# caki35/UNet-Torch

Measured on AMD Instinct MI355X. Metric: images/sec training step, 4-level U-Net 1ch→2cls 512×512, at 1/2/4/8 MI355X, higher is better.
Workload: dtype f16

## Files before the change

include/unetmi.h:

```cpp
#ifndef UNETMI_H
#define UNETMI_H
#include <stddef.h>
#include <stdint.h>

#ifdef __cplusplus
extern "C" {
#endif

typedef void* umi_stream_t;

enum { UMI_F32 = 0, UMI_F16 = 1 };
enum { UMI_OK = 0, UMI_ERR_BADARG = -1, UMI_ERR_UNSUPPORTED = -2, UMI_ERR_WORKSPACE = -3 };
enum { UMI_CONV_UPSAMPLE2 = 1,
       UMI_CONV_FORCE_GENERIC = 2,
       UMI_CONV_DGRAD_STRIDED = 4,
       UMI_CONV_ACCUMULATE = 8,
       UMI_CONV_F32_MFMA = 16,
       UMI_CONV_F32_MFMA_1X1 = 32,
       UMI_CONV_F32_MFMA_2X2 = 64   };

int umi_version(void);
const char* umi_arch(void);

int umi_tune_conv3x3_impl(int impl);

int umi_pack_kn(const float* src, void* dst, int T, int K, int N, long st, long sk, long sn,
                int flip_t, int Kpad, int Npad, int dtype, umi_stream_t stream);

int umi_pack_kn8(const float* src, void* dst, int T, int K, int N, long st, long sk, long sn,
                 int flip_t, int Kpad, int Npad, int dtype, umi_stream_t stream);

int umi_conv_fwd(const void* x, int ldx, const void* tx, const void* wp, const float* bias,
                 void* y, int ldy, float* stat_part,
                 int N, int H, int W, int Ci, int Co, int R, int S, int stride, int pad,
                 int Ho, int Wo, int off_h, int off_w, int out_H, int out_W,
                 int in_dtype, int out_dtype, int flags, umi_stream_t stream);
int umi_linear_fused(const void* x, int ldx, const void* wp8, const float* bias, void* y, int ldy, long M, int Ci, int Co,
                     int epi, float p, unsigned seed, const unsigned* seed_dev, void* mask, const void* aux, int ldaux,
                     void* y2, int ldy2, int dtype, umi_stream_t stream);

int umi_conv_fwd_plan(int N, int H, int W, int Ci, int Co, int R, int S, int stride, int pad,
                      int ldx, int ldy, int in_dtype, int out_dtype, int flags, int has_bias,
                      int* layout, int* stat_rows);

int umi_bn_finalize(const float* stat_part, int rows, int C, double count,
                    const float* gamma, const float* beta, float eps, float momentum,
                    float* running_mean, float* running_var,
                    void* tx_out, float* rstd_out, umi_stream_t stream);
int umi_bn_stat_sums(const float* stat_part, int rows, int C, double* sums, umi_stream_t stream);
int umi_bn_finalize_sums(const double* sums, int C, double count,
                         const float* gamma, const float* beta, float eps, float momentum,
                         float* running_mean, float* running_var,
                         void* tx_out, float* rstd_out, umi_stream_t stream);

int umi_pool2_fwd(const void* x, int ldx, const void* tx, void* y, int ldy,
                  int N, int H, int W, int C, int dtype, umi_stream_t stream);
int umi_pool2_bwd(const void* dpool, int lddp, const void* x, int ldx, const void* tx,
                  void* da, int ldda, int accumulate,
                  int N, int H, int W, int C, int dtype, umi_stream_t stream);

size_t umi_bn_bwd_ws_bytes(long M, int C);
int umi_bn_bwd_reduce(const void* da, int ldda, const void* y, int ldy, const void* tx,
                      const float* rstd, float* sum_dz, float* sum_dzx,
                      long M, int C, int dtype, void* ws, size_t ws_bytes, umi_stream_t stream);
int umi_bn_bwd_apply(void* da, int ldda, const void* y, int ldy, const void* tx,
                     const float* rstd, const float* sum_dz, const float* sum_dzx,
                     long M, int C, int dtype, umi_stream_t stream);
int umi_bn_bwd_apply_count(void* da, int ldda, const void* y, int ldy, const void* tx,
                           const float* rstd, const float* sum_dz, const float* sum_dzx,
                           long M, long count, int C, int dtype, umi_stream_t stream);

int umi_conv_dgrad_bnred(const void* dy, int lddy, const void* wp8, void* da, int ldda, const void* ybn, int ldybn,
                         const void* txbn, const float* rstd, float* part, int N, int H, int W, int Ci, int Co,
                         int dtype, umi_stream_t stream);

int umi_conv_gather_bnred_rows(int N, int H, int W, int Ci, int Co, int R, int S, int stride, int pad, int Ho, int Wo,
                               int ldx, int ldy, int dtype, int flags);
int umi_conv_gather_bnred(const void* x, int ldx, const void* wp8, void* y, int ldy, const void* ybn, int ldybn,
                          const void* txbn, const float* rstd, float* part, int N, int H, int W, int Ci, int Co, int R, int S,
                          int stride, int pad, int Ho, int Wo, int dtype, int flags, umi_stream_t stream);

int umi_head_dgrad_bnred_rows(long P, int Ci, int Co, int ldda, int dtype);
int umi_head_dgrad_bnred(const void* dl, int lddl, const void* wp, void* da, int ldda, const void* ybn, int ldybn,
                         const void* txbn, const float* rstd, float* part, long P, int Ci, int Co, int dtype,
                         umi_stream_t stream);
size_t umi_head_bwd_fused_ws_bytes(long P, int Ci, int Co);
int umi_head_bwd_fused(const void* dl, int lddl, const void* wp, void* da, int ldda, const void* ybn, int ldybn,
                       const void* txbn, const float* rstd, float* part, float* dW, long s_co, long s_ci, float out_scale,
                       void* ws, size_t ws_bytes, long P, int Ci, int Co, int dtype, umi_stream_t stream);

int umi_conv3x3_fwd_act(const void* x, int ldx, const void* tx, const void* wp8, const void* out_tx, void* y, int ldy,
                        int N, int H, int W, int Ci, int Co, int dtype, umi_stream_t stream);
int umi_bn_stats_rows(long M, int C);
int umi_bn_stats(const void* x, int ldx, float* part, long M, int C, int dtype, umi_stream_t stream);
int umi_pool2_bwd_bnred_stat_rows(int N, int H, int W, int C);
int umi_pool2_bwd_bnred(const void* dpool, int lddp, const void* x, int ldx, const void* tx, const float* rstd, void* da,
                        int ldda, int accumulate, float* part, int N, int H, int W, int C, int dtype, umi_stream_t stream);
int umi_bn_bwd_from_partials(const float* part, int rows, int C, float* sum_dz, float* sum_dzx, umi_stream_t stream);

size_t umi_conv_wgrad_ws_bytes(int N, int Ho, int Wo, int Ci, int Co, int R, int S, int dtype, int flags);
int umi_conv_wgrad(const void* x, int ldx, const void* txa, const void* dy, int lddy, const void* txb,
                   float* dW, long s_co, long s_ci, long s_t, float out_scale,
                   int N, int H, int W, int Ci, int Co, int R, int S, int stride, int pad,
                   int Ho, int Wo, int dtype, int flags, void* ws, size_t ws_bytes, umi_stream_t stream);
typedef struct umi_wgrad_pending {
    const float* part;
    float* dW;
    long s_co, s_ci, s_t;
    float scale;
    int splits, RS, Ci, Co;
} umi_wgrad_pending;
int umi_conv_wgrad_deferred(const void* x, int ldx, const void* txa, const void* dy, int lddy, const void* txb,
                            float* dW, long s_co, long s_ci, long s_t, float out_scale, int N, int H, int W, int Ci, int Co,
                            int R, int S, int stride, int pad, int Ho, int Wo, int dtype, int flags, void* ws, size_t ws_bytes,
                            umi_wgrad_pending* out, umi_stream_t stream);
int umi_wgrad_reduce_group(int n, const void* items , umi_stream_t stream);
int umi_conv_wgrad_bias(const void* x, int ldx, const void* dy, int lddy, const void* txb, float* dW, long s_co, long s_ci,
                        long s_t, float* dbias, float out_scale, int N, int H, int W, int Ci, int Co, int Ho, int Wo, int dtype,
                        int flags, void* ws, size_t ws_bytes, umi_wgrad_pending* out, umi_stream_t stream);
int umi_conv_wgrad_group(int n, const void* const* x, int ldx, const void* const* dy, int lddy, float* const* dW, long s_co,
                         long s_ci, float out_scale, long M, int Ci, int Co, int dtype, umi_stream_t stream);
int umi_conv_wgrad_bnapply(const void* x, int ldx, const void* txa, const void* da, int ldda, const void* y, int ldy,
                           const void* tx_bn, const float* rstd, const float* sum_dz, const float* sum_dzx, void* dz,
                           int lddz, float* dW, long s_co, long s_ci, long s_t, float out_scale, int N, int H, int W,
                           int Ci, int Co, int R, int S, int stride, int pad, int dtype, int flags, void* ws,
                           size_t ws_bytes, umi_stream_t stream);
int umi_conv_wgrad_bnapply_count(const void* x, int ldx, const void* txa, const void* da, int ldda, const void* y, int ldy,
                                 const void* tx_bn, const float* rstd, const float* sum_dz, const float* sum_dzx, void* dz,
                                 int lddz, float* dW, long s_co, long s_ci, long s_t, float out_scale, int N, int H, int W,
                                 int Ci, int Co, int R, int S, int stride, int pad, int dtype, int flags, long count, void* ws,
                                 size_t ws_bytes, umi_stream_t stream);

size_t umi_colsum_ws_bytes(long M, int C);
int umi_colsum(const void* x, int ldx, float* out, float out_scale, long M, int C, int dtype,
               void* ws, size_t ws_bytes, umi_stream_t stream);
int umi_colsum_group(int n, const void* const* xs, int ldx, float* const* outs, float out_scale, long M, int C, int dtype,
                     void* ws, size_t ws_bytes, umi_stream_t stream);

int umi_materialize_nchw(const void* x, int ldx, const void* tx, float* y_nchw,
                         int N, int H, int W, int C, int dtype, umi_stream_t stream);


int umi_wstd_fwd(const float* w, float* wstd, float* rstd, int Co, int K, float eps, umi_stream_t stream);
int umi_wstd_bwd(const float* wstd, const float* rstd, const float* g, float* dw, int Co, int K, umi_stream_t stream);
typedef struct umi_wstd_desc {
    const float* w;
    float* ws;
    float* rstd;
    long off;
    int Co, K;
    float eps;
    int blk0;
    float* dw;
} umi_wstd_desc;
int umi_wstd_fwd_multi(const void* descs, int n_desc, int total_rows, umi_stream_t stream);
int umi_wstd_bwd_multi(const void* descs, int n_desc, int total_rows, const float* g_base, float* dw_base, umi_stream_t stream);

size_t umi_gn_fwd_ws_bytes(int N, long HW, int C);
int umi_gn_fwd(const void* x, int ldx, const float* gamma, const float* beta, const void* res, int ldr, void* y, int ldy,
               float* mean, float* rstd, int relu, int N, long HW, int C, int G, float eps, int dtype,
               void* ws, size_t ws_bytes, umi_stream_t stream);
size_t umi_gn_bwd_ws_bytes(int N, long HW, int C, int G);
int umi_gn_bwd(const void* dy, int lddy, const void* y, int ldy, const void* x, int ldx, const float* mean,
               const float* rstd, const float* gamma, int relu, void* dx, int lddx, void* dres, int lddr,
               float* dgamma, float* dbeta, float out_scale, int N, long HW, int C, int G, int dtype,
               void* ws, size_t ws_bytes, float* part_out, umi_stream_t stream);
int umi_gn_param_grads_group(int n, const float* const* parts, const int* Cs, int N, float* const* dgammas,
                             float* const* dbetas, float out_scale, umi_stream_t stream);

int umi_pool3s2_fwd(const void* x, int ldx, void* y, int ldy, void* idx, int N, int H, int W, int C, int dtype,
                    umi_stream_t stream);
int umi_pool3s2_bwd(const void* dy, int lddy, const void* x, int ldx, const void* idx, void* dx, int lddx, int N, int H, int W,
                    int C, int dtype, umi_stream_t stream);

int umi_ln_fwd(const void* x, int ldx, const float* gamma, const float* beta, void* y, int ldy, float* mean, float* rstd,
               long M, int C, float eps, int dtype, umi_stream_t stream);
size_t umi_ln_bwd_ws_bytes(long M, int C);
int umi_ln_bwd(const void* dy, int lddy, const void* x, int ldx, const float* gamma, const float* mean,
               const float* rstd, void* dx, int lddx, float* dgamma, float* dbeta, float out_scale, long M, int C,
               int dtype, void* ws, size_t ws_bytes, int* rows_out, umi_stream_t stream);

int umi_elementwise(int mode, const void* x, int ldx, const void* g, int ldg, void* y, int ldy, long M, int C,
                    long bcast_rows, int dtype, umi_stream_t stream);

int umi_dropout(const void* x, int ldx, void* y, int ldy, void* mask, int backward, float p, unsigned seed, long M, int C,
                int dtype, const void* tx, const unsigned* seed_dev, umi_stream_t stream);
int umi_dropout_fused(const void* x, int ldx, void* y, int ldy, void* mask, int backward, float p, unsigned seed, long M, int C,
                      int dtype, const unsigned* seed_dev, const void* aux, int ldaux, int gelu, umi_stream_t stream);

int umi_attn_fwd(const void* q, const void* k, const void* v, int ld, void* o, int ldo, float* lse, int B, int N, int heads,
                 int D, int dtype, umi_stream_t stream);
int umi_attn_bwd(const void* q, const void* k, const void* v, int ld, const void* o, const void* dO, int ldo,
                 const float* lse, void* dq, void* dk, void* dv, int ldd, float* delta, int B, int N, int heads, int D,
                 int dtype, umi_stream_t stream);
enum { UMI_ATTN_F32_MFMA = 1  };
int umi_attn_fwd_flags(const void* q, const void* k, const void* v, int ld, void* o, int ldo, float* lse, int B, int N, int heads,
// ... 196 lines not shown
```

unet-torch_amd/csrc/conv1x1_mfma.hip:

```cpp
#include "kernels.h"
#include <stdlib.h>
#include <string.h>

typedef _Float16 half8 __attribute__((ext_vector_type(8)));
typedef _Float16 half4 __attribute__((ext_vector_type(4)));
typedef float floatx16 __attribute__((ext_vector_type(16)));
typedef float floatx4 __attribute__((ext_vector_type(4)));
typedef unsigned u32x4 __attribute__((ext_vector_type(4)));

namespace {

constexpr int OUT_UPS_TAPS_MAX = 49;

constexpr int CK = 64;
constexpr int ROWB = 160;

struct Geo {
    int h, w;
    int Hs, Ws, soy, sox;
    int Hd, Wd, doy, dox;
    int S, stride, pad, frac;
    int accum;
    int epi;
    float drop_p;
// ... 264 lines not shown
            for (int k = 0; k < NPS; ++k) {
                const int p = p0 + k * PSTEP;
                if (m0 + p < M && col_ok) {
                    const int2 pi = dense ? make_int2(0, 0) : pixinfo[p];
                    const long drow = dense ? (m0 + p) : ((long)pi.x * geo.Hd + (pi.y >> 16)) * geo.Wd + (pi.y & 0xffff);
                    ybv[k] = *reinterpret_cast<const half8*>(geo.aux + drow * geo.ldaux + cop);
                }
            }
        }
#pragma unroll
        for (int k = 0; k < NPS; ++k) {
            const int p = p0 + k * PSTEP;
            if (m0 + p >= M || !col_ok) break;
            const int2 pi = dense ? make_int2(0, 0) : pixinfo[p];
            int yy = pi.y >> 16, xx = pi.y & 0xffff;
            if (OUT_UPS) {
                yy = 2 * yy + tdy;
                xx = 2 * xx + tdx;
                if (yy < 0 || yy >= geo.Hd || xx < 0 || xx >= geo.Wd) continue;
            }
            uint4 v = *reinterpret_cast<const uint4*>(smem + p * ERS + j * 16);
            half_t* dst = dense ? y + (m0 + p) * ldy + co : y + ((long)((long)pi.x * geo.Hd + yy) * geo.Wd + xx) * ldy + co;
            if (geo.accum) {
                const half8 o = *reinterpret_cast<const half8*>(dst);
                v = __builtin_bit_cast(uint4, (half8)(o + __builtin_bit_cast(half8, v)));
            }
            if (geo.epi == 1 || geo.epi == 2) {
                const long e0 = (m0 + p) * (long)Ntot_ + cop;
                const unsigned seed = geo.seed + (geo.seed_dev ? geo.seed_dev[0] * 0x9E3779B9u : 0u);
                const float scale = 1.f / (1.f - geo.drop_p);
                const half8 xv = __builtin_bit_cast(half8, v);
                half8 av, o;
                if (geo.epi == 2) av = *reinterpret_cast<const half8*>(geo.aux + (m0 + p) * geo.ldaux + cop);
                unsigned long long mk = 0;
#pragma unroll
                for (int jj = 0; jj < 8; ++jj) {
                    const long e = e0 + jj;
                    const float u = (umi_stream_hash32((unsigned)e, seed ^ (unsigned)(e >> 32)) >> 8) * (1.f / 16777216.f);
                    const unsigned k = u >= geo.drop_p;
                    mk |= (unsigned long long)k << (8 * jj);
                    float f = (float)xv[jj];
                    if (geo.epi == 1) f = umi_gelu(f);
                    f = k ? f * scale : 0.f;
                    if (geo.epi == 2) f += (float)av[jj];
                    o[jj] = (half_t)f;
                }
                *reinterpret_cast<unsigned long long*>(geo.mask + e0) = mk;
                if (geo.epi == 1) *reinterpret_cast<half8*>(geo.y2 + (m0 + p) * geo.ldy2 + cop) = o;
                else v = __builtin_bit_cast(uint4, o);
            }
#ifdef UMI_X_NOSTORE
            if (v.x == 0x12345678u)
#endif
            *reinterpret_cast<uint4*>(dst) = v;
            if (geo.epi == 3 && !OUT_UPS) {
                const half8 yv = ybv[k];
                const half8 hv = __builtin_bit_cast(half8, v);
#pragma unroll
                for (int jj = 0; jj < 8; ++jj) {
                    const float yy_ = (float)yv[jj];
                    const float dz = umi_tx_pre(yy_, bt[jj]) > bt[jj].w ? (float)hv[jj] : 0.f;
                    bs[jj] += dz;
                    bq[jj] = fmaf(dz, (yy_ - bt[jj].x) * brs[jj], bq[jj]);
                }
            }
        }
        if (geo.epi == 3) {
            __syncthreads();
            float* rs_ = reinterpret_cast<float*>(smem);
#pragma unroll
            for (int jj = 0; jj < 8; ++jj) {
                rs_[(0 * PSTEP + p0) * BN + j * 8 + jj] = bs[jj];
                rs_[(1 * PSTEP + p0) * BN + j * 8 + jj] = bq[jj];
            }
            __syncthreads();
            if (tid < 2 * BN) {
                const int which = tid / BN, cc = tid % BN;
                float a = 0.f;
#pragma unroll 8
                for (int k = 0; k < PSTEP; ++k) a += rs_[(which * PSTEP + k) * BN + cc];
                if (c0 + cc < Ntot_) geo.bn_part[((m0 / P) * 2 + which) * Ntot_ + c0 + cc] = a;
            }
        }
    }
}

template <int P, int BN>
int launch(bool s2d, bool ups, const void* x, int ldx, const void* tx, const void* wp8, const float* bias, void* y,
           int ldy, long M, int Kc, int Nc, int Ntot, int ntaps, Geo geo, hipStream_t s) {
    const int n_co = (Ntot + BN - 1) / BN;
    const long nblk = ((M + P - 1) / P) * n_co;
    dim3 grid((unsigned)((nblk + 7) / 8 * 8)), block(256);
#define GO(S2D, UPS, HT)                                                                                          \
    hipLaunchKernelGGL((conv1x1_mfma_kernel<P, BN, S2D, UPS, HT>), grid, block, 0, s, (const half_t*)x, ldx,      \
                       (const float4*)tx, (const half_t*)wp8, bias, (half_t*)y, ldy, M, Kc, Nc, n_co, ntaps, geo, nblk)
    if (s2d) { if (tx) GO(true, false, true); else GO(true, false, false); }
    else if (ups) { if (tx) GO(false, true, true); else GO(false, true, false); }
    else { if (tx) GO(false, false, true); else GO(false, false, false); }
#undef GO
    UMI_LAUNCH_CHECK();
    return UMI_OK;
}

}

static int umi_conv1x1_mode(int R, int S, int stride, int pad, int flags) {
    if (flags & UMI_CONV_UPSAMPLE2) return (R == 2 && S == 2) ? 1 : -1;
    if (R * S > 49 || pad < 0 || pad >= 1 << 20) return -1;
    if (flags & UMI_CONV_DGRAD_STRIDED) return stride >= 1 ? 2 : -1;
    if (R == 1 && S == 1 && stride == 1 && pad == 0) return 0;
    if (stride >= 2) return 2;
    return -1;
}

bool umi_conv1x1_mfma_ok(const ConvFwdProblem& p) {
    if (p.flags & UMI_CONV_FORCE_GENERIC) return false;
    if (p.in_dtype != UMI_F16 || p.out_dtype != UMI_F16) return false;
    const int mode = umi_conv1x1_mode(p.R, p.S, p.stride, p.pad, p.flags);
    if (mode < 0) return false;
    if (p.ldx % 8 || p.ldy % 8) return false;
    if ((long)(OUT_UPS_TAPS_MAX) * p.Ci * p.Co * 2 >= 0x7FFFFFF0L) return false;
    if (mode == 0) return p.Ci % 8 == 0 && p.Co % 8 == 0 && p.Ci >= 16 && p.Co >= 16;
    if (p.Ci % 64 || p.Co % 64) return false;
    if (2L * p.H * p.W * p.ldx * 2 >= 0x7FFFFFF0L) return false;
    return true;
}

static void c1_pick_tile(long M, int Ntot, int* P, int* BN) {
    const bool bn128 = Ntot % 128 == 0;
    const long want = 300;
    const long b_256_128 = ((M + 255) / 256) * (Ntot / 128), b_128_128 = ((M + 127) / 128) * (Ntot / 128);
    const long b_256_64 = ((M + 255) / 256) * (Ntot / 64);
    if (const char* e = getenv("UMI_C1_TILE")) {
        const int p_ = atoi(e), bn_ = strchr(e, 'x') ? atoi(strchr(e, 'x') + 1) : 0;
        if ((p_ == 256 || p_ == 128) && ((bn_ == 128 && bn128) || bn_ == 64)) { *P = p_; *BN = bn_; return; }
    }
    if (bn128 && b_256_128 >= want) { *P = 256; *BN = 128; return; }
    if (b_256_64 >= want) { *P = 256; *BN = 64; return; }
    if (bn128 && b_128_128 >= want) { *P = 128; *BN = 128; return; }
    *P = 128; *BN = 64;
}
int umi_conv1x1_bnred_rows(long M, int Ntot) {
    int P, BN;
    c1_pick_tile(M, Ntot, &P, &BN);
    return (int)((M + P - 1) / P);
}

int umi_conv1x1_mfma(const ConvFwdProblem& p, const void* x, const void* tx, const void* wp8, const float* bias, void* y,
                     int off_h, int off_w, int out_H, int out_W, hipStream_t s, const UmiLinearEpi* epi) {
    const int N = p.N, H = p.H, W = p.W, Ci = p.Ci, Co = p.Co, Ho = p.Ho, Wo = p.Wo, ldx = p.ldx, ldy = p.ldy, flags = p.flags;
    const int mode = umi_conv1x1_mode(p.R, p.S, p.stride, p.pad, flags);
    if (epi && epi->mode && epi->mode != 3 && (mode != 0 || (flags & UMI_CONV_ACCUMULATE) || Co % 8)) return UMI_ERR_UNSUPPORTED;
    if (epi && epi->mode == 3 && (mode == 1 || Co % 8)) return UMI_ERR_UNSUPPORTED;
    Geo geo;
    long M;
    int Kc = Ci, Nc = Co, Ntot = Co, ntaps = 1;
    if (mode == 0) {
        geo = Geo{H, W, H, W, 0, 0, H, W, 0, 0, 1, 1, 0, 0};
        M = (long)N * H * W;
    } else if (mode == 1) {
        geo = Geo{H, W, H, W, 0, 0, out_H, out_W, off_h, off_w, 1, 1, 0, 0};
        M = (long)N * H * W;
        Ntot = 4 * Co;
    } else {
        geo = Geo{Ho, Wo, H, W, 0, 0, Ho, Wo, 0, 0, p.S, p.stride, p.pad, (flags & UMI_CONV_DGRAD_STRIDED) ? 1 : 0};
        M = (long)N * Ho * Wo;
        ntaps = p.R * p.S;
    }
    geo.accum = (flags & UMI_CONV_ACCUMULATE) ? 1 : 0;
    geo.epi = 0; geo.drop_p = 0.f; geo.seed = 0; geo.seed_dev = nullptr; geo.mask = nullptr; geo.aux = nullptr; geo.ldaux = 0;
    geo.y2 = nullptr; geo.ldy2 = 0; geo.bn_tx = nullptr; geo.bn_rstd = nullptr; geo.bn_part = nullptr;
    if (epi && epi->mode) {
        geo.epi = epi->mode; geo.drop_p = epi->p; geo.seed = epi->seed; geo.seed_dev = epi->seed_dev;
        geo.mask = (unsigned char*)epi->mask; geo.aux = (const half_t*)epi->aux; geo.ldaux = epi->ldaux;
        geo.y2 = (half_t*)epi->y2; geo.ldy2 = epi->ldy2;
        geo.bn_tx = (const float4*)epi->bn_tx; geo.bn_rstd = epi->bn_rstd; geo.bn_part = epi->bn_part;
    }
#define GO(P_, BN_) return launch<P_, BN_>(mode == 2, mode == 1, x, ldx, tx, wp8, bias, y, ldy, M, Kc, Nc, Ntot, ntaps, geo, s)
    int tp, tbn;
    c1_pick_tile(M, Ntot, &tp, &tbn);
    if (tp == 256 && tbn == 128) GO(256, 128);
    if (tp == 256) GO(256, 64);
    if (tbn == 128) GO(128, 128);
    GO(128, 64);
#undef GO
}
```

unet-torch_amd/csrc/kernels.h:

```cpp
#pragma once
#include "common.h"

struct ConvFwdProblem {
    int N, H, W, Ci, Co, R, S, stride, pad, Ho, Wo, ldx, ldy, in_dtype, out_dtype, flags;
    bool has_tx, has_bias, has_stats;
};
enum ConvFwdPath { FWD_MFMA3X3_F32, FWD_GEMM_F32, FWD_CONVT_F32, FWD_MFMA3X3, FWD_MFMA1X1, FWD_STEM, FWD_HEAD, FWD_SMALLK, FWD_ROOT, FWD_HEAD3, FWD_GENERIC };

bool umi_conv3x3_f32_mfma_ok(const ConvFwdProblem& p);
bool umi_gemm_f32_mfma_ok(const ConvFwdProblem& p);
bool umi_convt_f32_mfma_ok(const ConvFwdProblem& p);
bool umi_conv3x3_mfma_ok(const ConvFwdProblem& p);
bool umi_conv1x1_mfma_ok(const ConvFwdProblem& p);
bool umi_stem_fwd_ok(const ConvFwdProblem& p);
bool umi_head_fwd_ok(const ConvFwdProblem& p);
bool umi_smallk_fwd_ok(const ConvFwdProblem& p);
bool umi_root_fwd_ok(const ConvFwdProblem& p);
bool umi_head3_fwd_ok(const ConvFwdProblem& p);

constexpr int UMI_CONV_F32_OPT_IN = UMI_CONV_F32_MFMA | UMI_CONV_F32_MFMA_1X1 | UMI_CONV_F32_MFMA_2X2;
inline ConvFwdPath umi_conv_fwd_path(const ConvFwdProblem& p) {
    if (p.flags & UMI_CONV_F32_OPT_IN) {
        if (umi_conv3x3_f32_mfma_ok(p)) return FWD_MFMA3X3_F32;
        if (umi_gemm_f32_mfma_ok(p)) return FWD_GEMM_F32;
        if (umi_convt_f32_mfma_ok(p)) return FWD_CONVT_F32;
        ConvFwdProblem q = p;
        q.flags &= ~UMI_CONV_F32_OPT_IN;
        return umi_conv_fwd_path(q);
    }
    if (p.flags & UMI_CONV_DGRAD_STRIDED)
        return umi_conv1x1_mfma_ok(p) ? FWD_MFMA1X1 : FWD_GENERIC;
    if (umi_conv3x3_mfma_ok(p)) return FWD_MFMA3X3;
    if (umi_conv1x1_mfma_ok(p)) return FWD_MFMA1X1;
    if (umi_stem_fwd_ok(p)) return FWD_STEM;
    if ((!p.has_stats || p.out_dtype == UMI_F16) && umi_head_fwd_ok(p)) return FWD_HEAD;
    if (p.has_stats) return FWD_GENERIC;
    if (umi_smallk_fwd_ok(p)) return FWD_SMALLK;
    if (umi_root_fwd_ok(p)) return FWD_ROOT;
    if (umi_head3_fwd_ok(p)) return FWD_HEAD3;
    return FWD_GENERIC;
}

struct UmiLinearEpi {
    int mode; float p; unsigned seed; const unsigned* seed_dev; void* mask; const void* aux; int ldaux; void* y2; int ldy2;
    const void* bn_tx; const float* bn_rstd; float* bn_part;
};

int umi_conv_fwd_generic(const ConvFwdProblem& p, const void* x, const void* tx, const void* wp, const float* bias, void* y,
                         float* stat_part, int off_h, int off_w, int out_H, int out_W, hipStream_t s);
int umi_conv3x3_f32_mfma_stat_rows(int N, int H, int W);
int umi_conv3x3_f32_mfma(const ConvFwdProblem& p, const void* x, const void* tx, const void* wp, void* y, float* stat_part,
                         hipStream_t s);
int umi_gemm_f32_mfma_stat_rows(long M);
int umi_gemm_f32_mfma(const ConvFwdProblem& p, const void* x, const void* tx, const void* wp, const float* bias, void* y,
                      float* stat_part, hipStream_t s);
int umi_convt_f32_mfma(const ConvFwdProblem& p, const void* x, const void* tx, const void* wp, const float* bias, void* y,
                       int off_h, int off_w, int out_H, int out_W, hipStream_t s);
int umi_conv3x3_mfma_stat_rows(int N, int H, int W, int Co);
int umi_conv3x3_mfma(const ConvFwdProblem& p, const void* x, const void* tx, const void* wp8, void* y, float* stat_part,
                     hipStream_t s);
int umi_conv3x3_mfma_bnred(const ConvFwdProblem& p, const void* dy, const void* wp8, void* da, const void* ybn, int ldybn,
                           const void* txbn, const float* rstd, float* part, hipStream_t s);
int umi_conv3x3_mfma_act(const ConvFwdProblem& p, const void* x, const void* tx, const void* wp8, const void* out_tx, void* y,
                         hipStream_t s);
int umi_conv1x1_bnred_rows(long M, int Ntot);
int umi_conv1x1_mfma(const ConvFwdProblem& p, const void* x, const void* tx, const void* wp8, const float* bias, void* y,
                     int off_h, int off_w, int out_H, int out_W, hipStream_t s, const UmiLinearEpi* epi = nullptr);
int umi_stem_stat_rows(int N, int H, int W);
int umi_stem_fwd(const ConvFwdProblem& p, const void* x, const void* tx, const void* wp, void* y, float* part, hipStream_t s);
int umi_head_stat_rows(long P, int Ci);
int umi_head_fwd(const ConvFwdProblem& p, const void* x, const void* tx, const void* wp, const float* bias, void* y, float* part,
                 hipStream_t s);
int umi_smallk_fwd(const ConvFwdProblem& p, const void* x, const void* wp, void* y, hipStream_t s);
int umi_smallk_bnred_rows(long P, int Co);
int umi_smallk_fwd_bnred(const void* x, int ldx, const void* wp, void* y, int ldy, const void* ybn, int ldybn, const void* txbn,
                         const float* rstd, float* part, long P, int Ci, int Co, hipStream_t s, float* dW = nullptr, long s_co = 0,
                         long s_ci = 0, float out_scale = 1.f, void* ws = nullptr, size_t ws_bytes = 0);
int umi_root_fwd(const ConvFwdProblem& p, const void* x, const void* wp, void* y, hipStream_t s);
int umi_head3_fwd(const ConvFwdProblem& p, const void* x, const void* tx, const void* wp, const float* bias, void* y,
                  hipStream_t s);

struct WgradProblem {
    int N, H, W, Ci, Co, R, S, stride, pad, Ho, Wo, ldx, lddy, dtype, flags;
    bool has_txa, has_txb;
};
struct WgradOut {
    float* dW; long s_co, s_ci, s_t; float out_scale;
    void* ws; size_t ws_bytes;
    umi_wgrad_pending* defer;
    float* convT_bias;
};
struct WgradBnApply { const void* y; int ldy; const void* tx_bn; const float *rstd, *sum_dz, *sum_dzx; void* dz; int lddz;
                      long count; };
enum WgradPath { WGRAD_MFMA3X3_F32, WGRAD_GEMM_F32, WGRAD_CONVT_F32, WGRAD_MFMA3X3, WGRAD_MFMA1X1, WGRAD_T, WGRAD_GATHER, WGRAD_STEM, WGRAD_HEAD, WGRAD_ROOT, WGRAD_HEAD3, WGRAD_GENERIC };

bool umi_wgrad3x3_f32_mfma_ok(const WgradProblem& p);
bool umi_wgrad_gemm_f32_mfma_ok(const WgradProblem& p);
bool umi_wgrad_convt_f32_mfma_ok(const WgradProblem& p);
bool umi_wgrad3x3_mfma_ok(const WgradProblem& p);
bool umi_wgrad1x1_mfma_ok(const WgradProblem& p);
bool umi_wgradT_mfma_ok(const WgradProblem& p);
bool umi_wgrad_gather_mfma_ok(const WgradProblem& p);
bool umi_stem_wgrad_ok(const WgradProblem& p);
bool umi_head_wgrad_ok(const WgradProblem& p);
bool umi_root_wgrad_ok(const WgradProblem& p);
bool umi_head3_wgrad_ok(const WgradProblem& p);

inline WgradPath umi_conv_wgrad_path(const WgradProblem& p) {
    if (p.flags & UMI_CONV_F32_OPT_IN) {
        if (umi_wgrad3x3_f32_mfma_ok(p)) return WGRAD_MFMA3X3_F32;
        if (umi_wgrad_gemm_f32_mfma_ok(p)) return WGRAD_GEMM_F32;
        if (umi_wgrad_convt_f32_mfma_ok(p)) return WGRAD_CONVT_F32;
        WgradProblem q = p;
        q.flags &= ~UMI_CONV_F32_OPT_IN;
        return umi_conv_wgrad_path(q);
    }
    if (umi_wgrad3x3_mfma_ok(p)) return WGRAD_MFMA3X3;
    if (umi_wgrad1x1_mfma_ok(p)) return WGRAD_MFMA1X1;
    if (umi_wgradT_mfma_ok(p)) return WGRAD_T;
    if (umi_wgrad_gather_mfma_ok(p)) return WGRAD_GATHER;
    if (umi_stem_wgrad_ok(p)) return WGRAD_STEM;
    if (umi_head_wgrad_ok(p)) return WGRAD_HEAD;
    if (umi_root_wgrad_ok(p)) return WGRAD_ROOT;
    if (umi_head3_wgrad_ok(p)) return WGRAD_HEAD3;
    return WGRAD_GENERIC;
}

size_t umi_wgrad3x3_f32_mfma_ws_bound(const WgradProblem& p);
size_t umi_wgrad_gemm_f32_mfma_ws_bound(const WgradProblem& p);
size_t umi_wgrad_convt_f32_mfma_ws_bound(const WgradProblem& p);
size_t umi_wgrad3x3_mfma_ws_bound(const WgradProblem& p);
size_t umi_wgrad1x1_mfma_ws_bound(const WgradProblem& p);
size_t umi_wgradT_mfma_ws_bound(const WgradProblem& p);
size_t umi_wgrad_gather_mfma_ws_bound(const WgradProblem& p);
size_t umi_stem_wgrad_ws_bound(const WgradProblem& p);
size_t umi_head_wgrad_ws_bound(const WgradProblem& p);
size_t umi_root_wgrad_ws_bound(const WgradProblem& p);
size_t umi_head3_wgrad_ws_bound(const WgradProblem& p);
size_t umi_conv_wgrad_generic_ws_bound(const WgradProblem& p);

int umi_wgrad3x3_f32_mfma(const WgradProblem& p, const void* x, const void* txa, const void* dy, const WgradOut& o, hipStream_t s);
int umi_wgrad_gemm_f32_mfma(const WgradProblem& p, const void* x, const void* txa, const void* dy, const WgradOut& o, hipStream_t s);
int umi_wgrad_convt_f32_mfma(const WgradProblem& p, const void* x, const void* txa, const void* dy, const void* txb,
                             const WgradOut& o, hipStream_t s);
int umi_wgrad3x3_mfma(const WgradProblem& p, const void* x, const void* txa, const void* dy, const WgradOut& o, hipStream_t s,
                      const WgradBnApply* bna = nullptr);
int umi_wgrad1x1_mfma(const WgradProblem& p, const void* x, const void* txa, const void* dy, const WgradOut& o, hipStream_t s);
int umi_wgradT_mfma(const WgradProblem& p, const void* x, const void* dy, const void* txb, const WgradOut& o, hipStream_t s);
int umi_wgrad_gather_mfma(const WgradProblem& p, const void* x, const void* txa, const void* dy, const WgradOut& o, hipStream_t s);
int umi_stem_wgrad(const WgradProblem& p, const void* x, const void* txa, const void* dy, const WgradOut& o, hipStream_t s,
                   const WgradBnApply* bna = nullptr);
int umi_head_wgrad(const WgradProblem& p, const void* x, const void* txa, const void* dy, const WgradOut& o, hipStream_t s);
int umi_root_wgrad(const WgradProblem& p, const void* x, const void* dy, const WgradOut& o, hipStream_t s);
int umi_head3_wgrad(const WgradProblem& p, const void* x, const void* txa, const void* dy, const WgradOut& o, hipStream_t s);
int umi_conv_wgrad_generic(const WgradProblem& p, const void* x, const void* txa, const void* dy, const void* txb,
                           const WgradOut& o, hipStream_t s);
int umi_wgrad1x1_mfma_group(int n, const void* const* x, int ldx, const void* const* dy, int lddy, float* const* dW, long s_co,
                            long s_ci, float out_scale, long M, int Ci, int Co, hipStream_t s);

void umi_launch_wgrad_reduce(int splits, int RS, int Ci, int Co, const WgradOut& o, hipStream_t s);
void umi_launch_reduce_rows2(const float* ws, int rows, int C, float* out0, float* out1, float scale, hipStream_t s);

int umi_bn_bwd_rpb_f16v(long M);
int umi_colsum_rows_f16v(long M, int C);
bool umi_colsum_f16v(const void* x, int ldx, float* ws, long M, int C, hipStream_t s);
bool umi_colsum_group_f16v(int n, const void* const* xs, int ldx, float* const* outs, float scale, float* ws, long M, int C,
                           hipStream_t s);
bool umi_bn_stats_f16v(const void* x, int ldx, float* part, long M, int C, hipStream_t s);
bool umi_bn_bwd_reduce1_f16v(const void* da, int ldda, const void* y, int ldy, const void* tx, const float* rstd, float* ws,
                             long M, int C, hipStream_t s);
bool umi_bn_bwd_apply_f16v(void* da, int ldda, const void* y, int ldy, const void* tx, const float* rstd,
                           const float* sum_dz, const float* sum_dzx, long M, long count, int C, hipStream_t s);
bool umi_pool2_fwd_f16v(const void* x, int ldx, const void* tx, void* y, int ldy, int N, int H, int W, int C,
                        hipStream_t s);
bool umi_pool2_bwd_f16v(const void* dp, int lddp, const void* x, int ldx, const void* tx, void* da, int ldda,
                        int accumulate, int N, int H, int W, int C, hipStream_t s);
int umi_pool2_bwd_bnred_rows(int N, int H, int W, int C);
bool umi_pool2_bwd_bnred_f16v(const void* dp, int lddp, const void* x, int ldx, const void* tx, const float* rstd, void* da,
                              int ldda, int accumulate, float* part, int N, int H, int W, int C, hipStream_t s);

int umi_gn_splits(int N, long HW);
bool umi_gn_fwd_f16v(const void* x, int ldx, const float* gamma, const float* beta, const void* res, int ldr, void* y, int ldy,
                     float* mean, float* rstd, int relu, int N, long HW, int C, int G, float eps, float* ws, hipStream_t s);
bool umi_gn_bwd_f16v(const void* dy, int lddy, const void* y, int ldy, const void* x, int ldx, const float* mean,
                     const float* rstd, const float* gamma, int relu, void* dx, int lddx, void* dres, int lddr, int N, long HW,
                     int C, int G, float* part, float* ws, hipStream_t s);
void umi_gn_param_grads_launch(int n, const float* const* parts, const int* Cs, int N, float* const* dgammas, float* const* dbetas,
                               float scale, hipStream_t s);

bool umi_ew_f16v(int mode, const void* x, int ldx, const void* g, int ldg, void* y, int ldy, long M, int C, long bcast_rows,
                 hipStream_t s);
bool umi_pool3s2_fwd_f16v(const void* x, int ldx, void* y, int ldy, void* idx, int N, int H, int W, int C, hipStream_t s);
bool umi_pool3s2_bwd_f16v(const void* dy, int lddy, const void* idx, void* dx, int lddx, int N, int H, int W, int C, hipStream_t s);
bool umi_dropout_f16v(const void* x, int ldx, void* y, int ldy, void* mask, int backward, float p, unsigned seed, long M, int C,
                      const void* tx, const unsigned* seed_dev, hipStream_t s);
bool umi_dropout_fused_f16v(const void* x, int ldx, void* y, int ldy, void* mask, int backward, float p, unsigned seed, long M,
                            int C, const unsigned* seed_dev, const void* aux, int ldaux, int gelu, hipStream_t s);
int umi_ln_bwd_rows_f16v();
bool umi_ln_bwd_f16v(const void* dy, int lddy, const void* x, int ldx, const float* gamma, const float* mean, const float* rstd,
                     void* dx, int lddx, float* part, long M, int C, hipStream_t s);
bool umi_bilinear2x_f16v(const void* x, int ldx, const void* tx, void* y, int ldy, int backward, int N, int H, int W, int C,
                         hipStream_t s);

bool umi_attn_mfma_ok(int D, int ld, int ldo, int dtype, const void* a, const void* b, const void* c);
int umi_attn_fwd_mfma(const void* q, const void* k, const void* v, int ld, void* o, int ldo, float* lse, int B, int N, int Hh,
                      const UmiAttnDrop* drop, hipStream_t s);
int umi_attn_bwd_mfma(const void* q, const void* k, const void* v, int ld, const void* o, const void* dO, int ldo,
                      const float* lse, void* dq, void* dk, void* dv, int ldd, float* delta, int B, int N, int Hh,
                      const UmiAttnDrop* drop, hipStream_t s);

bool umi_attn_f32_mfma_ok(int D, int ld, int ldo, int ldd, int dtype, int flags, uintptr_t ptrs);
int umi_attn_fwd_f32_mfma(const void* q, const void* k, const void* v, int ld, void* o, int ldo, float* lse, int B, int N, int Hh,
                          const UmiAttnDrop* drop, hipStream_t s);
int umi_attn_bwd_f32_mfma(const void* q, const void* k, const void* v, int ld, const void* o, const void* dO, int ldo,
                          const float* lse, void* dq, void* dk, void* dv, int ldd, float* delta, int B, int N, int Hh,
                          const UmiAttnDrop* drop, hipStream_t s);
```

Baseline: 745.4.

## Add persistent weight-resident streaming kernel for 2x2 transposed-conv upsample

Adds a persistent kernel for the 2x2 stride-2 transposed convolution (upsample) forward path. Each workgroup keeps one output-channel panel of weights resident in LDS, then streams pixel tiles through it with register-prefetched, double-buffered input loads and MFMA 16x16x32 f16 compute. Results are staged through per-wave LDS and written as 2x2 scattered stores. This avoids reloading weights per tile and overlaps global loads with compute, at the cost of a large LDS footprint, one workgroup per CU, and a fixed residency guess of 256 workgroups. It is enabled by default for eligible shapes (Ci of 64, 128 or 256) and can be disabled through an environment variable.

```diff
diff --git a/include/unetmi.h b/include/unetmi.h
--- a/include/unetmi.h
+++ b/include/unetmi.h
@@ -42,6 +42,8 @@
 int umi_conv_fwd_plan(int N, int H, int W, int Ci, int Co, int R, int S, int stride, int pad,
                       int ldx, int ldy, int in_dtype, int out_dtype, int flags, int has_bias,
                       int* layout, int* stat_rows);
+int umi_convt_stream_plan(int N, int H, int W, int Ci, int Co, int R, int S, int ldx, int ldy, int in_dtype, int out_dtype, int flags,
+                          int out_H, int out_W, int off_h, int off_w, int* panels, int* wgs_per_panel, int* tile_pixels);
 
 int umi_bn_finalize(const float* stat_part, int rows, int C, double count,
                     const float* gamma, const float* beta, float eps, float momentum,
diff --git a/unet-torch_amd/csrc/conv1x1_mfma.hip b/unet-torch_amd/csrc/conv1x1_mfma.hip
--- a/unet-torch_amd/csrc/conv1x1_mfma.hip
+++ b/unet-torch_amd/csrc/conv1x1_mfma.hip
@@ -440,6 +440,10 @@
     const int mode = umi_conv1x1_mode(p.R, p.S, p.stride, p.pad, flags);
     if (epi && epi->mode && epi->mode != 3 && (mode != 0 || (flags & UMI_CONV_ACCUMULATE) || Co % 8)) return UMI_ERR_UNSUPPORTED;
     if (epi && epi->mode == 3 && (mode == 1 || Co % 8)) return UMI_ERR_UNSUPPORTED;
+    if (mode == 1 && !(epi && epi->mode) && umi_convt_stream_ok(p, off_h, off_w, out_H, out_W)) {
+        const char* e = getenv("UMI_CONVT_STREAM");
+        if (!(e && e[0] == '0')) return umi_convt_stream(p, x, tx, wp8, bias, y, off_h, off_w, out_H, out_W, s);
+    }
     Geo geo;
     long M;
     int Kc = Ci, Nc = Co, Ntot = Co, ntaps = 1;
diff --git a/unet-torch_amd/csrc/convt_stream.hip b/unet-torch_amd/csrc/convt_stream.hip
--- /dev/null
+++ b/unet-torch_amd/csrc/convt_stream.hip
@@ -0,0 +1,343 @@
+#include "kernels.h"
+#include <stdlib.h>
+#include <type_traits>
+
+typedef _Float16 half8 __attribute__((ext_vector_type(8)));
+typedef _Float16 half4 __attribute__((ext_vector_type(4)));
+typedef float floatx4 __attribute__((ext_vector_type(4)));
+typedef unsigned u32x4 __attribute__((ext_vector_type(4)));
+
+namespace {
+
+constexpr int ROWB = 160;
+constexpr int RESIDENT = 256;
+constexpr int MIN_TILES = 4;
+constexpr unsigned OOB = 0x7FFFFFFFu;
+
+template <int KC> struct Cfg {
+    static constexpr int PW = KC <= 2 ? 256 : 128;
+    static constexpr int PT = 64;
+    static constexpr int CW = 64;
+    static constexpr int WN = PW / CW, WM = 2;
+    static constexpr int NW = WN * WM, NTHR = NW * 64;
+    static constexpr bool DOUBLE = KC <= 2;
+    static constexpr int NCT = CW / 16, NPT = PT / (16 * WM);
+    static constexpr int WBYTES = KC * PW * ROWB, XBYTES = KC * PT * ROWB;
+    static constexpr int ERS = CW * 2 + 16, EBYTES = 16 * ERS;
+    static constexpr int SMEM = WBYTES + (DOUBLE ? 2 : 1) * XBYTES + NW * EBYTES + 2 * PT * (int)sizeof(int2) + 16;
+    static constexpr int NPIECE = PT * KC * 8 / NTHR;
+    static constexpr int NWPIECE = PW * KC * 8 / NTHR;
+};
+
+#ifdef UMI_XS_NOMFMA
+#define UMI_XS_MMA(c_, a_, b_) do { if ((ks | ct | i) == 0) c_[0] += (float)a_[0] * (float)b_[0]; else asm volatile("" :: "v"(a_), "v"(b_)); } while (0)
+#else
+#define UMI_XS_MMA(c_, a_, b_) c_ = __builtin_amdgcn_mfma_f32_16x16x32_f16(a_, b_, c_, 0, 0, 0)
+#endif
+#ifdef UMI_XS_NOSTORE
+#define UMI_XS_STORE_OK (pi.y == 0x12345678)
+#else
+#define UMI_XS_STORE_OK true
+#endif
+#ifdef UMI_XS_NOLOAD
+#define UMI_XS_LOAD_OK (ldx == 0x12345678)
+#else
+#define UMI_XS_LOAD_OK true
+#endif
+
+struct StreamGeo {
+    int hw, h, w;
+    int Hd, Wd, doy, dox;
+    int panels, wgs;
+    int ntiles;
+    int nimg;
+    int dn, dy, dx;
+};
+
+template <int KC, bool HAS_TX>
+__global__ __launch_bounds__(Cfg<KC>::NTHR, 1) void convt_stream_kernel(
+    const half_t* __restrict__ x, int ldx, const float4* __restrict__ tx, const half_t* __restrict__ wp8,
+    const float* __restrict__ bias, half_t* __restrict__ y, int ldy, long M, int Nc, StreamGeo g) {
+    using C = Cfg<KC>;
+    constexpr int Kc = KC * 64, NTHR = C::NTHR, NXB = C::DOUBLE ? 2 : 1;
+    extern __shared__ __attribute__((aligned(16))) unsigned char smem[];
+    const int tid = threadIdx.x, lane = tid & 63, wave = tid >> 6;
+    const int wn = wave % C::WN, wm = wave / C::WN;
+    const int lrow = lane & 15, lgrp = lane >> 4;
+    const int q = (int)blockIdx.x >> 3;
+    const int panel = q % g.panels, slot = (q / g.panels) * 8 + ((int)blockIdx.x & 7);
+    if (slot >= g.wgs) return;
+
+    unsigned char* const wl = smem;
+    unsigned char* const xl = smem + C::WBYTES;
+    unsigned char* const el = smem + C::WBYTES + NXB * C::XBYTES + wave * C::EBYTES;
+    int2* const pinfo = reinterpret_cast<int2*>(smem + C::WBYTES + NXB * C::XBYTES + C::NW * C::EBYTES);
+    int* const tinfo = reinterpret_cast<int*>(pinfo + 2 * C::PT);
+
+    {
+        const __amdgpu_buffer_rsrc_t wrs = __builtin_amdgcn_make_buffer_rsrc((void*)wp8, 0, (int)(4L * Kc * Nc * 2), 0x00020000);
+        u32x4 wr[C::NWPIECE];
+#pragma unroll
+        for (int j = 0; j < C::NWPIECE; ++j) {
+            const int idx = tid + NTHR * j, col = idx % C::PW, k8 = idx / C::PW;
+            const int cop = panel * C::PW + col, tap = cop / Nc, co = cop - tap * Nc;
+            wr[j] = __builtin_bit_cast(u32x4, __builtin_amdgcn_raw_buffer_load_b128(
+                wrs, (unsigned)((((long)tap * (Kc >> 3) + k8) * Nc + co) * 16), 0, 0));
+        }
+#pragma unroll
+        for (int j = 0; j < C::NWPIECE; ++j) {
+            const int idx = tid + NTHR * j, col = idx % C::PW, k8 = idx / C::PW;
+            *reinterpret_cast<u32x4*>(wl + ((k8 >> 3) * C::PW + col) * ROWB + (k8 & 7) * 16) = wr[j];
+        }
+    }
+    const int c8 = tid % (KC * 8);
+    float4 t8[8];
+    if (HAS_TX) {
+#pragma unroll
+        for (int j = 0; j < 8; ++j) t8[j] = tx[c8 * 8 + j];
+    }
+    const int cop0 = panel * C::PW + wn * C::CW, tapw = cop0 / Nc, cow = cop0 - tapw * Nc;
+    const int lane_off = (((tapw >> 1) * g.Wd + (tapw & 1)) * ldy + cow + (lane % (C::CW / 8)) * 8) * 2;
+    float bv[C::NCT][4];
+#pragma unroll
+    for (int ct = 0; ct < C::NCT; ++ct)
+#pragma unroll
+        for (int j = 0; j < 4; ++j) bv[ct][j] = bias ? bias[cow + ct * 16 + lgrp * 4 + j] : 0.f;
+
+    u32x4 xr[2][C::NPIECE];
+#define UMI_ISSUE(t_, S_)                                                                                            \
+    do {                                                                                                          \
+        const int tt = (t_);                                                                                      \
+        const bool live = tt < g.ntiles;                                                                          \
+        const long m0 = (long)tt * C::PT;                                                                         \
+        const long left = M - m0;                                                                                 \
+        const int rows = live ? (left < C::PT ? (int)left : C::PT) : 0;                                           \
+        const __amdgpu_buffer_rsrc_t xrs = __builtin_amdgcn_make_buffer_rsrc(                                     \
+            (void*)(x + (live ? m0 * ldx : 0)), 0, live ? ((rows - 1) * ldx + Kc) * 2 : 0, 0x00020000);           \
+        _Pragma("unroll") for (int j = 0; j < C::NPIECE; ++j) {                                                   \
+            const int pix = (tid + NTHR * j) / (KC * 8);                                                          \
+            xr[S_][j] = __builtin_bit_cast(u32x4, __builtin_amdgcn_raw_buffer_load_b128(                           \
+                xrs, UMI_XS_LOAD_OK ? (unsigned)((pix * ldx + c8 * 8) * 2) : OOB, 0, 0));                         \
+        }                                                                                                         \
+    } while (0)
+#define UMI_STAGE(t_, S_, b_)                                                                                      \
+    do {                                                                                                          \
+        const int tt = (t_);                                                                                      \
+        const long m0 = (long)tt * C::PT;                                                                         \
+        unsigned char* const xb = xl + (C::DOUBLE ? (b_) : 0) * C::XBYTES;                                        \
+        _Pragma("unroll") for (int j = 0; j < C::NPIECE; ++j) {                                                   \
+            const int pix = (tid + NTHR * j) / (KC * 8);                                                          \
+            if (HAS_TX && tt < g.ntiles && m0 + pix < M)                                                          \
+                xr[S_][j] = __builtin_bit_cast(u32x4, umi_tx8(__builtin_bit_cast(half8, xr[S_][j]), t8));         \
+            *reinterpret_cast<u32x4*>(xb + ((c8 >> 3) * C::PT + pix) * ROWB + (c8 & 7) * 16) = xr[S_][j];         \
+        }                                                                                                         \
+    } while (0)
+
+    unsigned pm = 0;
+    int pn = 0, py = 0, px_ = 0;
+    if (tid < C::PT) {
+        pm = (unsigned)slot * C::PT + tid;
+        pn = (int)(pm / (unsigned)g.hw);
+        const unsigned r = pm - (unsigned)pn * (unsigned)g.hw;
+        py = (int)(r / (unsigned)g.w);
+        px_ = (int)(r - (unsigned)py * (unsigned)g.w);
+    }
+#define UMI_PINFO(b_)                                                                                              \
+    do {                                                                                                          \
+        if (tid < C::PT) {                                                                                        \
+            const int n0t = __builtin_amdgcn_readfirstlane(pn);              \
+            int2 pi = make_int2(0, 0);                            \
+            if ((long)pm < M) {                                                                                   \
+                const int y0 = 2 * py + g.doy, x0 = 2 * px_ + g.dox;                                              \
+                const long off = (((long)(pn - n0t) * g.Hd + y0) * g.Wd + x0) * ldy * 2;                          \
+                int mask = 0;                                                                                     \
+                _Pragma("unroll") for (int k = 0; k < 4; ++k) {                                                   \
+                    const long offk = off + ((long)(k >> 1) * g.Wd + (k & 1)) * ldy * 2;                          \
+                    if (y0 + (k >> 1) < g.Hd && x0 + (k & 1) < g.Wd && offk + Nc * 2 <= 0x7FFFFFF0L) mask |= 1 << k; \
+                }                                                                                                 \
+                pi = make_int2((int)off, mask);                                                                   \
+            }                                                                                                     \
+            pinfo[(b_) * C::PT + tid] = pi;                                                                       \
+            if (tid == 0) tinfo[b_] = n0t;                                                                        \
+            pm += (unsigned)g.wgs * C::PT;                                                                        \
+            px_ += g.dx; if (px_ >= g.w) { px_ -= g.w; ++py; }                                                    \
+            py += g.dy; if (py >= g.h) { py -= g.h; ++pn; }                                                       \
+            pn += g.dn;                                                                                           \
+        }                                                                                                         \
+    } while (0)
+
+    const int b_base = (wm * C::NPT * 16 + lrow) * ROWB + lgrp * 16;
+    const int a_base = (wn * C::CW + lrow) * ROWB + lgrp * 16;
+    const long yimg = (long)g.Hd * g.Wd * ldy;
+
+    auto tile = [&](const int t, auto par) {
+        constexpr int I = decltype(par)::value, buf = I;
+        UMI_ISSUE(t + 2 * g.wgs, I);
+        UMI_PINFO(I ^ 1);
+        __builtin_amdgcn_sched_barrier(0);
+        floatx4 acc[C::NCT][C::NPT];
+#pragma unroll
+        for (int a = 0; a < C::NCT; ++a)
+#pragma unroll
+            for (int b = 0; b < C::NPT; ++b)
+#pragma unroll
+                for (int r = 0; r < 4; ++r) acc[a][b][r] = 0.f;
+        const unsigned char* const xb = xl + (C::DOUBLE ? buf : 0) * C::XBYTES;
+        half8 af[2][C::NCT], bf[2][C::NPT];
+#define UMI_FRAGS(ks_)                                                                                             \
+        do {                                                                                                      \
+            const int kc = (ks_) >> 1, k2 = (ks_) & 1;                                                            \
+            _Pragma("unroll") for (int ct = 0; ct < C::NCT; ++ct)                                                 \
+                af[(ks_) & 1][ct] = *reinterpret_cast<const half8*>(wl + a_base + (kc * C::PW + ct * 16) * ROWB + k2 * 64); \
+            _Pragma("unroll") for (int i = 0; i < C::NPT; ++i)                                                    \
+                bf[(ks_) & 1][i] = *reinterpret_cast<const half8*>(xb + b_base + (kc * C::PT + i * 16) * ROWB + k2 * 64); \
+        } while (0)
+        UMI_FRAGS(0);
+        __builtin_amdgcn_sched_barrier(0);
+#pragma unroll
+        for (int ks = 0; ks < 2 * KC; ++ks) {
+            if (ks + 1 < 2 * KC) UMI_FRAGS(ks + 1);
+            __builtin_amdgcn_sched_barrier(0);
+#pragma unroll
+            for (int ct = 0; ct < C::NCT; ++ct)
+#pragma unroll
+                for (int i = 0; i < C::NPT; ++i)
+                    UMI_XS_MMA(acc[ct][i], af[ks & 1][ct], bf[ks & 1][i]);
+            __builtin_amdgcn_sched_barrier(0);
+        }
+#undef UMI_FRAGS
+
+        const int n0 = __builtin_amdgcn_readfirstlane(tinfo[buf]);
+        const long yleft = (((long)(g.nimg - n0) * g.Hd * g.Wd - 1) * ldy + Nc) * 2;
+        const __amdgpu_buffer_rsrc_t yrs = __builtin_amdgcn_make_buffer_rsrc(
+            (void*)(y + (long)n0 * yimg), 0, (int)(yleft > 0x7FFFFFF0L ? 0x7FFFFFF0L : yleft), 0x00020000);
+#pragma unroll
+        for (int pt = 0; pt < C::NPT; ++pt) {
+#pragma unroll
+            for (int ct = 0; ct < C::NCT; ++ct) {
+                half4 h;
+#pragma unroll
+                for (int j = 0; j < 4; ++j) h[j] = (half_t)(acc[ct][pt][j] + bv[ct][j]);
+                *reinterpret_cast<half4*>(el + lrow * C::ERS + (ct * 16 + lgrp * 4) * 2) = h;
+            }
+            __builtin_amdgcn_fence(__ATOMIC_RELEASE, "wavefront");
+            __builtin_amdgcn_wave_barrier();
+            __builtin_amdgcn_fence(__ATOMIC_ACQUIRE, "wavefront");
+            constexpr int PPR = C::CW / 8;
+#pragma unroll
+            for (int i = 0; i < 16 * PPR / 64; ++i) {
+                const int qd = lane + 64 * i, j = qd % PPR, px = qd / PPR;
+                const u32x4 v = *reinterpret_cast<const u32x4*>(el + px * C::ERS + j * 16);
+                const int2 pi = pinfo[buf * C::PT + wm * C::NPT * 16 + pt * 16 + px];
+                __builtin_amdgcn_raw_buffer_store_b128(v, yrs, (UMI_XS_STORE_OK && ((pi.y >> tapw) & 1)) ? (unsigned)(pi.x + lane_off) : OOB, 0, 0);
+            }
+            __builtin_amdgcn_fence(__ATOMIC_RELEASE, "wavefront");
+            __builtin_amdgcn_wave_barrier();
+            __builtin_amdgcn_fence(__ATOMIC_ACQUIRE, "wavefront");
+        }
+
+        if (!C::DOUBLE) __syncthreads();
+        UMI_STAGE(t + g.wgs, I ^ 1, I ^ 1);
+        __syncthreads();
+    };
+    UMI_ISSUE(slot, 0);
+    UMI_STAGE(slot, 0, 0);
+    UMI_PINFO(0);
+    UMI_ISSUE(slot + g.wgs, 1);
+    __syncthreads();
+    for (int t = slot; t < g.ntiles; t += 2 * g.wgs) {
+        tile(t, std::integral_constant<int, 0>());
+        if (t + g.wgs >= g.ntiles) break;
+        tile(t + g.wgs, std::integral_constant<int, 1>());
+    }
+#undef UMI_ISSUE
+#undef UMI_STAGE
+#undef UMI_PINFO
+}
+
+struct StreamPlan { int kc, pw, pt, panels, wgs, ntiles; };
+
+bool stream_plan(const ConvFwdProblem& p, int off_h, int off_w, int out_H, int out_W, StreamPlan* o) {
+    if (p.flags & ~UMI_CONV_UPSAMPLE2) return false;
+    if (!(p.flags & UMI_CONV_UPSAMPLE2) || p.R != 2 || p.S != 2) return false;
+    if (p.in_dtype != UMI_F16 || p.out_dtype != UMI_F16) return false;
+    if (p.N <= 0 || p.H <= 0 || p.W <= 0 || p.Ci <= 0 || p.Co <= 0 || out_H <= 0 || out_W <= 0 || off_h < 0 || off_w < 0) return false;
+    if (p.Ci % 64 || p.Co % 64) return false;
+    if (p.ldx % 8 || p.ldy % 8 || p.ldx < p.Ci || p.ldy < p.Co) return false;
+    const int kc = p.Ci / 64;
+    if (kc != 1 && kc != 2 && kc != 4) return false;
+    const int pw = kc <= 2 ? 256 : 128, pt = 64;
+    if ((4 * p.Co) % pw) return false;
+    if (4L * p.Ci * p.Co * 2 >= 0x7FFFFFF0L) return false;
+    const long M = (long)p.N * p.H * p.W;
+    if (2L * p.H * p.W * p.ldx * 2 >= 0x7FFFFFF0L || M >= (1L << 31)) return false;
+    if ((long)(pt / ((long)p.H * p.W) + 2) * out_H * out_W * p.ldy * 2 >= 0x7FFFFFF0L) return false;
+    const long nt = (M + pt - 1) / pt;
+    if (nt < MIN_TILES) return false;
+    const int panels = 4 * p.Co / pw;
+    if (panels > RESIDENT / 8) return false;
+    long wgs = RESIDENT / panels;
+    if (const char* e = getenv("UMI_CONVT_STREAM_WGS")) {
+        const int cap = atoi(e);
+        if (cap > 0 && cap < wgs) wgs = cap;
+    }
+    if (wgs > nt) wgs = nt;
+    o->kc = kc; o->pw = pw; o->pt = pt; o->panels = panels; o->wgs = (int)wgs; o->ntiles = (int)nt;
+    return true;
+}
+
+template <int KC>
+int launch(const StreamPlan& pl, const ConvFwdProblem& p, const void* x, const void* tx, const void* wp8, const float* bias, void* y,
+           int off_h, int off_w, int out_H, int out_W, hipStream_t s) {
+    constexpr int dyn = Cfg<KC>::SMEM;
+    static const int attr_rc = [] {
+        int a = (int)hipFuncSetAttribute((const void*)convt_stream_kernel<KC, true>, hipFuncAttributeMaxDynamicSharedMemorySize, dyn);
+        int b = (int)hipFuncSetAttribute((const void*)convt_stream_kernel<KC, false>, hipFuncAttributeMaxDynamicSharedMemorySize, dyn);
+        return a ? a : b;
+    }();
+    if (attr_rc) return attr_rc;
+    const long step = (long)pl.wgs * Cfg<KC>::PT, hw = (long)p.H * p.W;
+    const StreamGeo g{p.H * p.W, p.H, p.W, out_H, out_W, off_h, off_w, pl.panels, pl.wgs, pl.ntiles, p.N,
+                      (int)(step / hw), (int)(step % hw / p.W), (int)(step % hw % p.W)};
+    const long M = (long)p.N * p.H * p.W;
+    dim3 grid((unsigned)((pl.wgs + 7) / 8 * 8 * pl.panels)), block(Cfg<KC>::NTHR);
+    if (tx)
+        hipLaunchKernelGGL((convt_stream_kernel<KC, true>), grid, block, dyn, s, (const half_t*)x, p.ldx, (const float4*)tx,
+                           (const half_t*)wp8, bias, (half_t*)y, p.ldy, M, p.Co, g);
+    else
+        hipLaunchKernelGGL((convt_stream_kernel<KC, false>), grid, block, dyn, s, (const half_t*)x, p.ldx, (const float4*)tx,
+                           (const half_t*)wp8, bias, (half_t*)y, p.ldy, M, p.Co, g);
+    UMI_LAUNCH_CHECK();
+    return UMI_OK;
+}
+
+}
+
+bool umi_convt_stream_ok(const ConvFwdProblem& p, int off_h, int off_w, int out_H, int out_W) {
+    StreamPlan pl;
+    return stream_plan(p, off_h, off_w, out_H, out_W, &pl);
+}
+
+int umi_convt_stream(const ConvFwdProblem& p, const void* x, const void* tx, const void* wp8, const float* bias, void* y,
+                     int off_h, int off_w, int out_H, int out_W, hipStream_t s) {
+    StreamPlan pl;
+    if (!stream_plan(p, off_h, off_w, out_H, out_W, &pl)) return UMI_ERR_UNSUPPORTED;
+    if (((uintptr_t)x | (uintptr_t)y | (uintptr_t)wp8) & 15) return UMI_ERR_BADARG;
+    if (pl.kc == 1) return launch<1>(pl, p, x, tx, wp8, bias, y, off_h, off_w, out_H, out_W, s);
+    if (pl.kc == 2) return launch<2>(pl, p, x, tx, wp8, bias, y, off_h, off_w, out_H, out_W, s);
+    return launch<4>(pl, p, x, tx, wp8, bias, y, off_h, off_w, out_H, out_W, s);
+}
+
+extern "C" int umi_convt_stream_plan(int N, int H, int W, int Ci, int Co, int R, int S, int ldx, int ldy, int in_dtype, int out_dtype,
+                                     int flags, int out_H, int out_W, int off_h, int off_w, int* panels, int* wgs_per_panel,
+                                     int* tile_pixels) {
+    ConvFwdProblem p{};
+    p.N = N; p.H = H; p.W = W; p.Ci = Ci; p.Co = Co; p.R = R; p.S = S; p.stride = 2; p.pad = 0; p.Ho = H; p.Wo = W;
+    p.ldx = ldx; p.ldy = ldy; p.in_dtype = in_dtype; p.out_dtype = out_dtype; p.flags = flags;
+    StreamPlan pl;
+    if (!stream_plan(p, off_h, off_w, out_H, out_W, &pl)) return UMI_ERR_UNSUPPORTED;
+    if (panels) *panels = pl.panels;
+    if (wgs_per_panel) *wgs_per_panel = pl.wgs;
+    if (tile_pixels) *tile_pixels = pl.pt;
+    return UMI_OK;
+}
diff --git a/unet-torch_amd/csrc/kernels.h b/unet-torch_amd/csrc/kernels.h
--- a/unet-torch_amd/csrc/kernels.h
+++ b/unet-torch_amd/csrc/kernels.h
@@ -66,6 +66,9 @@
 int umi_conv1x1_bnred_rows(long M, int Ntot);
 int umi_conv1x1_mfma(const ConvFwdProblem& p, const void* x, const void* tx, const void* wp8, const float* bias, void* y,
                      int off_h, int off_w, int out_H, int out_W, hipStream_t s, const UmiLinearEpi* epi = nullptr);
+bool umi_convt_stream_ok(const ConvFwdProblem& p, int off_h, int off_w, int out_H, int out_W);
+int umi_convt_stream(const ConvFwdProblem& p, const void* x, const void* tx, const void* wp8, const float* bias, void* y,
+                     int off_h, int off_w, int out_H, int out_W, hipStream_t s);
 int umi_stem_stat_rows(int N, int H, int W);
 int umi_stem_fwd(const ConvFwdProblem& p, const void* x, const void* tx, const void* wp, void* y, float* part, hipStream_t s);
 int umi_head_stat_rows(long P, int Ci);
```

Result: no change. 749.7 (median of 6 runs) (+0.6%).
